# steineggerlab/Metabuli

Measured on AMD Instinct MI355X. Metric: Mreads/s classified (metabuli classify hot path, reads + index resident in HBM), higher is better.
Workload: dtype u64

## Files before the change

### include/mtb.h

```cpp
#ifndef MTB_H
#define MTB_H
#include <stddef.h>
#include <stdint.h>

#ifdef __cplusplus
extern "C" {
#endif

typedef enum {
    MTB_OK = 0,
    MTB_ERR_ARG = 1,
    MTB_ERR_IO = 2,
    MTB_ERR_DEVICE = 3,
    MTB_ERR_CAPACITY = 4,
    MTB_ERR_OOM = 5,
    MTB_ERR_UNSUPPORTED = 6
} mtb_status;

typedef struct { uint64_t value; uint64_t qinfo; } mtb_kmer;

typedef struct {
    uint64_t qinfo;
    int32_t  target_id;
    int32_t  species_id;
// ... 45 lines not shown
    uint32_t n_launch[MTB_NUM_KERNELS];
    uint64_t n_generic_reads;
    uint64_t n_slot_reads;
    uint64_t n_deferred_reads, n_many_reads, n_many_matches, n_many_kept;
    int32_t  join_variant, join_tuned;
    float    join_tune_ms[3];
    uint32_t join_tiles, join_tiles_windowed, join_tiles_outside;
} mtb_batch_stats;

typedef enum { MTB_JOIN_AUTO = 0, MTB_JOIN_Q1W6 = 1, MTB_JOIN_Q2W5 = 2, MTB_JOIN_WINDOW = 3 } mtb_join_variant;

const char *mtb_version(void);
const char *mtb_last_error(void);
void mtb_default_params(mtb_params *p);

mtb_status mtb_ctx_create(int device, void *stream, mtb_ctx **out);
void       mtb_ctx_destroy(mtb_ctx *);
mtb_status mtb_ctx_sync(mtb_ctx *);
mtb_status mtb_ctx_set_profiling(mtb_ctx *, int on);
mtb_status mtb_ctx_set_streams(mtb_ctx *, int n);
mtb_status mtb_ctx_set_workspace_limit(mtb_ctx *, uint64_t bytes);
mtb_status mtb_ctx_set_placement_probe(mtb_ctx *, int on);
mtb_status mtb_ctx_set_join_variant(mtb_ctx *, int variant);
mtb_status mtb_ctx_set_option(mtb_ctx *, const char *name, const char *value);
uint32_t   mtb_ctx_last_sub_batches(const mtb_ctx *);
uint64_t   mtb_ctx_last_scratch_bytes(const mtb_ctx *);

mtb_status mtb_index_open(mtb_ctx *, const char *dbdir, const char *taxonomy_dir,
                          mtb_params *params, mtb_index **out);
mtb_status mtb_index_open_stats(const mtb_index *, uint64_t *out4);
mtb_status mtb_index_from_device(mtb_ctx *, uint64_t *d_values, uint32_t *d_info,
                                 uint64_t n_targets, const char *taxonomy_dir,
                                 const int32_t *taxid_list, size_t n_taxids,
                                 const mtb_params *params, mtb_index **out);
mtb_status mtb_index_clone(mtb_index *src, mtb_ctx *dst_ctx, mtb_index **out);
typedef struct {
    uint8_t  values_handle[64], info_handle[64], dir_handle[64], dirbase_handle[64];
    uint64_t values_off, info_off, dir_off, dirbase_off;
    uint64_t n_targets;
    uint32_t dir_buckets, info_mask;
    int32_t  dir_depth, packed, has_info, match_last, device;
    int64_t  exporter_pid;
    uint64_t values_ptr, info_ptr, dir_ptr, dirbase_ptr;
} mtb_index_share;
mtb_status mtb_index_export(mtb_index *src, mtb_index_share *out);
mtb_status mtb_index_import(mtb_ctx *, const mtb_index_share *, const char *taxonomy_dir, const int32_t *taxid_list, size_t n_taxids,
// ... 164 lines not shown
```

### metabuli_amd/__init__.py

```python
from __future__ import annotations

import ctypes as C
import os
import subprocess

import numpy as np

_HERE = os.path.dirname(os.path.abspath(__file__))
_CSRC = os.path.join(_HERE, "csrc")
LIB_PATH = os.environ.get("MTB_LIB") or os.path.join(_CSRC, "libmtb.so")

kmer_dt = np.dtype([("value", "<u8"), ("qinfo", "<u8")])
match_dt = np.dtype([("qinfo", "<u8"), ("target_id", "<i4"), ("species_id", "<i4"), ("dna", "<u4"),
                     ("reh", "<u2"), ("ham", "u1"), ("pad", "u1")])
result_dt = np.dtype([("classification", "<i4"), ("score", "<f4"), ("qlen", "<i4"), ("qlen2", "<i4"),
                      ("is_classified", "u1"), ("flag", "u1"), ("n_taxcnt", "<u2"), ("taxcnt_off", "<u4")])

block_dt = np.dtype([("seq", "<u4"), ("strand", "<i4"), ("start", "<u8"), ("end", "<u8")])

MTB_OK, MTB_ERR_ARG, MTB_ERR_IO, MTB_ERR_DEVICE, MTB_ERR_CAPACITY, MTB_ERR_OOM, MTB_ERR_UNSUPPORTED = range(7)


class Params(C.Structure):
    _fields_ = [("seq_mode", C.c_int32), ("syncmer", C.c_int32), ("smer_len", C.c_int32),
# ... 112 lines not shown
        _chk(self.L.mtb_ctx_create(C.c_int(device), C.c_void_p(stream), C.byref(h)))
        self.h = h

    def close(self):
        if self.h:
            self.L.mtb_ctx_destroy(self.h)
            self.h = None

    def sync(self):
        _chk(self.L.mtb_ctx_sync(self.h))

    def set_profiling(self, on):
        _chk(self.L.mtb_ctx_set_profiling(self.h, C.c_int(1 if on else 0)))

    def set_placement_probe(self, on):
        _chk(self.L.mtb_ctx_set_placement_probe(self.h, C.c_int(1 if on else 0)))

    def set_workspace_limit(self, nbytes):
        _chk(self.L.mtb_ctx_set_workspace_limit(self.h, C.c_uint64(int(nbytes))))

    def set_join_variant(self, name):
        _chk(self.L.mtb_ctx_set_join_variant(self.h, C.c_int({"auto": 0, "q1w6": 1, "q2w5": 2, "window": 3}[name])))

    def set_option(self, name, value):
        _chk(self.L.mtb_ctx_set_option(self.h, name.encode(), None if value is None else str(value).encode()))

    @property
    def last_sub_batches(self):
        self.L.mtb_ctx_last_sub_batches.restype = C.c_uint32
        return int(self.L.mtb_ctx_last_sub_batches(self.h))

    @property
    def last_scratch_bytes(self):
        self.L.mtb_ctx_last_scratch_bytes.restype = C.c_uint64
        return int(self.L.mtb_ctx_last_scratch_bytes(self.h))

    def set_streams(self, n):
        _chk(self.L.mtb_ctx_set_streams(self.h, C.c_int(n)))

    def open_index(self, dbdir, params, taxonomy_dir=None):
        h = C.c_void_p()
        _chk(self.L.mtb_index_open(self.h, dbdir.encode(), taxonomy_dir.encode() if taxonomy_dir else None,
                                   C.byref(params), C.byref(h)))
        return Index(self, h)

    def clone_index(self, src):
# ... 461 lines not shown
```

### metabuli_amd/csrc/kernels_sort.h

```cpp
#ifndef MTB_KERNELS_SORT_H
#define MTB_KERNELS_SORT_H
#include "dev_util.h"
#include "kernels_scan.h"
#include "mtb_core.h"

#define MTB_SORT_TILE 2048
#ifndef MTB_SORT_ITEMS
#define MTB_SORT_ITEMS 8
#endif

template <int MODE>
__device__ __forceinline__ uint32_t radix_digit(uint64_t v, int shift) {
    if (MODE == 0) return (uint32_t)(v >> shift) & 255u;
    uint32_t two = (uint32_t)(v >> shift) & 1023u;
    uint32_t d = (two >> 5) * 21u + (two & 31u);
    return d < 511u ? d : 511u;
}

template <int NB, int MODE, int THREADS>
__global__ __launch_bounds__(THREADS) void k_radix_hist(const mtb_kmer *__restrict__ in, uint64_t n, int shift,
                                                         uint32_t *__restrict__ hist, uint32_t num_tiles) {
    __shared__ uint32_t s_h[NB];
    for (int b = threadIdx.x; b < NB; b += THREADS) s_h[b] = 0;
    __syncthreads();
    uint64_t base = (uint64_t)blockIdx.x * (THREADS * MTB_SORT_ITEMS);
#pragma unroll
    for (int r = 0; r < MTB_SORT_ITEMS; r++) {
        uint64_t i = base + (uint64_t)r * THREADS + threadIdx.x;
        if (i < n) atomicAdd(&s_h[radix_digit<MODE>(in[i].value, shift)], 1u);
    }
    __syncthreads();
    for (int b = threadIdx.x; b < NB; b += THREADS) hist[(uint64_t)b * num_tiles + blockIdx.x] = s_h[b];
}

#define MTB_HIST_GROUP 16
template <int NB, int THREADS, int TILE = THREADS * MTB_SORT_ITEMS>
__global__ __launch_bounds__(THREADS) void k_radix_hist_dig(const uint16_t *__restrict__ dig, uint64_t n, uint32_t *__restrict__ hist, uint32_t num_tiles) {
    static_assert(NB == THREADS, "one bin per thread");
    __shared__ uint32_t s_h[MTB_HIST_GROUP][NB];
    const uint32_t tile0 = blockIdx.x * MTB_HIST_GROUP;
#pragma unroll
    for (int g = 0; g < MTB_HIST_GROUP; g++) s_h[g][threadIdx.x] = 0;
    __syncthreads();
    for (int g = 0; g < MTB_HIST_GROUP; g++) {
        const uint64_t base = (uint64_t)(tile0 + g) * TILE;
        if (base >= n) break;
        if (TILE == THREADS * 8 && base + TILE <= n) {
            const uint4 q = *(const uint4 *)(dig + base + 8u * threadIdx.x);
            const uint32_t w[4] = {q.x, q.y, q.z, q.w};
#pragma unroll
            for (int k = 0; k < 4; k++) {
                const uint32_t d0 = w[k] & 0xFFFFu, d1 = w[k] >> 16;
                atomicAdd(&s_h[g][d0 < NB ? d0 : NB - 1], 1u);
                atomicAdd(&s_h[g][d1 < NB ? d1 : NB - 1], 1u);
            }
            continue;
        }
#pragma unroll
        for (int r = 0; r < TILE / THREADS; r++) {
            uint64_t i = base + (uint64_t)r * THREADS + threadIdx.x;
            if (i < n) { uint32_t d = dig[i]; atomicAdd(&s_h[g][d < NB ? d : NB - 1], 1u); }
        }
    }
    __syncthreads();
    uint32_t *row = hist + (uint64_t)threadIdx.x * num_tiles + tile0;
    if (tile0 + MTB_HIST_GROUP <= num_tiles && (((uint64_t)threadIdx.x * num_tiles + tile0) & 3u) == 0) {
#pragma unroll
        for (int g = 0; g < MTB_HIST_GROUP; g += 4) {
            uint4 v; v.x = s_h[g][threadIdx.x]; v.y = s_h[g + 1][threadIdx.x]; v.z = s_h[g + 2][threadIdx.x]; v.w = s_h[g + 3][threadIdx.x];
            *(uint4 *)(row + g) = v;
        }
    } else {
        for (int g = 0; g < MTB_HIST_GROUP && tile0 + g < num_tiles; g++) row[g] = s_h[g][threadIdx.x];
    }
}

#define MTB_SORT_NBKT 512
__device__ __forceinline__ uint32_t sort_tile_bucket(const uint32_t *__restrict__ first_tile, uint32_t t) {
    uint32_t lo = 0, hi = MTB_SORT_NBKT;
    while (hi - lo > 1) { const uint32_t mid = (lo + hi) >> 1; if (first_tile[mid] <= t) lo = mid; else hi = mid; }
    return lo;
}

template <int NB, int MODE, int THREADS>
__global__ __launch_bounds__(THREADS) void k_radix_scatter(const mtb_kmer *__restrict__ in, mtb_kmer *__restrict__ out,
                                                            uint64_t n, int shift, const uint32_t *__restrict__ tile_off,
                                                            uint32_t num_tiles, uint16_t *__restrict__ dig_out = nullptr, int next_shift = 0, int xcd_map = 1,
                                                            const uint32_t *__restrict__ plan = nullptr ) {
    constexpr int BITS = NB == 256 ? 8 : 9;
    constexpr int NW = THREADS / 64;
    constexpr int TILE = THREADS * MTB_SORT_ITEMS;
    static_assert(NB <= THREADS, "at least one thread per bin");
    __shared__ uint16_t s_cnt[NW][NB];
    __shared__ uint16_t s_start[NB];
    __shared__ uint32_t s_tmp[NW];
    __shared__ mtb_kmer s_buf[TILE];
    __shared__ uint32_t s_goff[NB];
    const uint32_t t = threadIdx.x, w = t >> 6, lane = t & 63u;
    if (plan) num_tiles = plan[513 + 512];
    const uint32_t per_xcd = (num_tiles + 7u) >> 3;
    const uint32_t tile = xcd_map ? (blockIdx.x & 7u) * per_xcd + (blockIdx.x >> 3) : blockIdx.x;
    if (tile >= num_tiles) return;
    uint64_t base = (uint64_t)tile * TILE;
    uint32_t my_off;
    if (plan) {
        const uint32_t *tfirst = plan + 513;
        const uint32_t b = sort_tile_bucket(tfirst, tile);
        const uint32_t j = tile - tfirst[b], ntb = tfirst[b + 1] - tfirst[b];
        base = (uint64_t)plan[b] + (uint64_t)j * TILE;
        n = plan[b + 1];
        my_off = t < NB ? tile_off[(uint64_t)512 * tfirst[b] + (uint64_t)t * ntb + j] : 0u;
    } else
    my_off = t < NB ? tile_off[(uint64_t)t * num_tiles + tile] : 0u;
    mtb_kmer e[MTB_SORT_ITEMS];
    uint32_t lrank[MTB_SORT_ITEMS];
    if (t < NB) {
#pragma unroll
        for (int k = 0; k < NW; k++) s_cnt[k][t] = 0;
    }
#pragma unroll
    for (int r = 0; r < MTB_SORT_ITEMS; r++) {
        uint64_t i = base + (uint64_t)w * (64 * MTB_SORT_ITEMS) + (uint64_t)r * 64 + lane;
        if (i < n) e[r] = in[i]; else { e[r].value = 0; e[r].qinfo = 0; }
    }
    __syncthreads();
#pragma unroll
    for (int r = 0; r < MTB_SORT_ITEMS; r++) {
        uint64_t i = base + (uint64_t)w * (64 * MTB_SORT_ITEMS) + (uint64_t)r * 64 + lane;
        bool valid = i < n;
        uint32_t d = radix_digit<MODE>(e[r].value, shift);
        uint64_t peers = __ballot(valid);
#pragma unroll
        for (int b = 0; b < BITS; b++) {
            bool bit = (d >> b) & 1u;
            uint64_t vote = __ballot(bit);
            peers &= bit ? vote : ~vote;
        }
        uint32_t rank_in_wave = (uint32_t)__popcll(peers & lanemask_lt());
        uint32_t before = s_cnt[w][d];
        __builtin_amdgcn_fence(__ATOMIC_ACQ_REL, "wavefront"); __builtin_amdgcn_wave_barrier();
        if (valid && rank_in_wave == 0) s_cnt[w][d] = (uint16_t)(before + (uint32_t)__popcll(peers));
        __builtin_amdgcn_fence(__ATOMIC_ACQ_REL, "wavefront"); __builtin_amdgcn_wave_barrier();
        lrank[r] = before + rank_in_wave;
    }
    __syncthreads();
    uint32_t run = 0;
    if (t < NB) {
#pragma unroll
        for (int k = 0; k < NW; k++) { uint32_t c = s_cnt[k][t]; s_cnt[k][t] = (uint16_t)run; run += c; }
    }
    uint32_t tot;
    uint32_t ex = block_exclusive_scan<uint32_t, NW>(run, s_tmp, &tot);
    if (t < NB) {
        s_start[t] = (uint16_t)ex;
        s_goff[t] = my_off - ex;
    }
    __syncthreads();
#pragma unroll
    for (int r = 0; r < MTB_SORT_ITEMS; r++) {
        uint64_t i = base + (uint64_t)w * (64 * MTB_SORT_ITEMS) + (uint64_t)r * 64 + lane;
        if (i < n) {
            uint32_t d = radix_digit<MODE>(e[r].value, shift);
            s_buf[(uint32_t)s_start[d] + s_cnt[w][d] + lrank[r]] = e[r];
        }
    }
    __syncthreads();
    uint32_t cnt = (uint32_t)((n - base) < TILE ? (n - base) : TILE);
    for (uint32_t i = t; i < cnt; i += THREADS) {
        mtb_kmer x = s_buf[i];
        uint32_t d = radix_digit<MODE>(x.value, shift);
        const uint64_t dst = (uint64_t)(s_goff[d] + i);
        out[dst] = x;
        if (dig_out) dig_out[dst] = (uint16_t)radix_digit<MODE>(x.value, next_shift);
    }
}

__global__ __launch_bounds__(512) void k_sort_plan(const uint32_t *__restrict__ scanned, uint32_t num_tiles, uint64_t n, uint32_t tile, uint32_t *__restrict__ plan) {
    __shared__ uint32_t s_tmp[8];
    const uint32_t b = threadIdx.x;
    const uint32_t start = scanned[(uint64_t)b * num_tiles];
    const uint32_t next = b + 1 < MTB_SORT_NBKT ? scanned[(uint64_t)(b + 1) * num_tiles] : (uint32_t)n;
    const uint32_t nt = (next - start + tile - 1) / tile;
    uint32_t tot;
    const uint32_t first = block_exclusive_scan<uint32_t, 8>(nt, s_tmp, &tot);
    plan[b] = start; plan[513 + b] = first;
    if (b == 0) { plan[512] = (uint32_t)n; plan[513 + 512] = tot; }
}
template <int NB, int THREADS, int TILE = THREADS * MTB_SORT_ITEMS>
__global__ __launch_bounds__(THREADS) void k_radix_hist_seg(const uint16_t *__restrict__ dig, const uint32_t *__restrict__ plan, uint32_t *__restrict__ hist) {
    static_assert(NB == THREADS, "one bin per thread");
    __shared__ uint32_t s_h[MTB_HIST_GROUP][NB];
    const uint32_t *bstart = plan, *tfirst = plan + 513;
    const uint32_t tiles = tfirst[512];
    const uint32_t tile0 = blockIdx.x * MTB_HIST_GROUP;
    if (tile0 >= tiles) return;
#pragma unroll
    for (int g = 0; g < MTB_HIST_GROUP; g++) s_h[g][threadIdx.x] = 0;
    __syncthreads();
    const uint32_t b0 = sort_tile_bucket(tfirst, tile0);
    uint32_t b = b0;
    for (int g = 0; g < MTB_HIST_GROUP; g++) {
        const uint32_t t = tile0 + g;
        if (t >= tiles) break;
        while (tfirst[b + 1] <= t) b++;
        const uint32_t base = bstart[b] + (t - tfirst[b]) * TILE;
        const uint32_t end = bstart[b + 1] < base + TILE ? bstart[b + 1] : base + TILE;
        if (TILE == THREADS * 8 && end == base + TILE && (base & 7u) == 0) {
            const uint4 q = *(const uint4 *)(dig + base + 8u * threadIdx.x);
            const uint32_t w[4] = {q.x, q.y, q.z, q.w};
#pragma unroll
            for (int k = 0; k < 4; k++) {
                const uint32_t d0 = w[k] & 0xFFFFu, d1 = w[k] >> 16;
                atomicAdd(&s_h[g][d0 < NB ? d0 : NB - 1], 1u);
                atomicAdd(&s_h[g][d1 < NB ? d1 : NB - 1], 1u);
            }
            continue;
        }
        const uint32_t a0 = base & ~7u;
        for (uint32_t ch = threadIdx.x; a0 + 8u * ch < end; ch += THREADS) {
            const uint32_t first = a0 + 8u * ch;
            const uint4 q = *(const uint4 *)(dig + first);
            const uint32_t w[4] = {q.x, q.y, q.z, q.w};
#pragma unroll
            for (int k = 0; k < 4; k++) {
                const uint32_t i0 = first + 2u * k, d0 = w[k] & 0xFFFFu, d1 = w[k] >> 16;
                if (i0 >= base && i0 < end) atomicAdd(&s_h[g][d0 < NB ? d0 : NB - 1], 1u);
                if (i0 + 1 >= base && i0 + 1 < end) atomicAdd(&s_h[g][d1 < NB ? d1 : NB - 1], 1u);
            }
        }
    }
    __syncthreads();
    const uint32_t last = tile0 + MTB_HIST_GROUP <= tiles ? tile0 + MTB_HIST_GROUP - 1 : tiles - 1;
    if (tfirst[b0 + 1] > last) {
        const uint32_t ntb = tfirst[b0 + 1] - tfirst[b0];
        uint32_t *row = hist + (uint64_t)512 * tfirst[b0] + (uint64_t)threadIdx.x * ntb + (tile0 - tfirst[b0]);
        for (uint32_t g = 0; g <= last - tile0; g++) row[g] = s_h[g][threadIdx.x];
    } else {
        uint32_t bb = b0;
        for (uint32_t g = 0; g <= last - tile0; g++) {
            const uint32_t t = tile0 + g;
            while (tfirst[bb + 1] <= t) bb++;
            const uint32_t ntb = tfirst[bb + 1] - tfirst[bb];
            hist[(uint64_t)512 * tfirst[bb] + (uint64_t)threadIdx.x * ntb + (t - tfirst[bb])] = s_h[g][threadIdx.x];
        }
    }
}

static inline uint64_t radix_hist_elems(uint64_t n, uint32_t bins = 256) { uint64_t tile = (uint64_t)bins * MTB_SORT_ITEMS; return (uint64_t)bins * ((n + tile - 1) / tile); }

static mtb_kmer *radix_sort_kmers(hipStream_t st, mtb_kmer *a, mtb_kmer *b, uint64_t n, int first_bit,
                                  uint32_t *hist, uint32_t *ws) {
    if (n == 0) return a;
    uint32_t tiles = (uint32_t)((n + MTB_SORT_TILE - 1) / MTB_SORT_TILE);
    mtb_kmer *src = a, *dst = b;
    for (int shift = first_bit; shift < 64; shift += 8) {
        hipLaunchKernelGGL((k_radix_hist<256, 0, 256>), dim3(tiles), dim3(256), 0, st, src, n, shift, hist, tiles);
        scan_launch<uint32_t, uint32_t, false>(st, hist, 256ull * tiles, false, hist, ws);
        hipLaunchKernelGGL((k_radix_scatter<256, 0, 256>), dim3((tiles + 7u) / 8u * 8u), dim3(256), 0, st, src, dst, n, shift, hist, tiles);
        mtb_kmer *tmp = src; src = dst; dst = tmp;
    }
    return src;
}

#endif
```

### metabuli_amd/csrc/mtb_api.hip

```cpp
#include <hip/hip_runtime.h>

#include <fcntl.h>
#include <limits.h>
#include <stdlib.h>
#include <sys/stat.h>
#include <unistd.h>

#include <atomic>
#include <chrono>
#include <condition_variable>
#include <mutex>
#include <functional>
#include <map>
#include <string>
#include <thread>
#include <vector>

#include "../../include/mtb.h"
#include "host_db.h"
#include "host/merge_plan.h"
#include "host/audit_plan.h"
#include "host/clade_filter.h"
#include "kernels_extract.h"
#include "kernels_extract_blocks.h"
// ... 90 lines not shown
    mtb_tables *d_tabs = nullptr;
    mtb_tables h_tabs;
    std::map<std::string, DevBuf> bufs;
    std::mutex bufs_mu;
    std::mutex reserve_mu;
    std::atomic<bool> reserve_cancel{false};
    uint64_t *d_scal = nullptr;
    unsigned long long *d_ovfctr = nullptr;
    uint64_t ovf_region = 0, ovf_max_region = 0;
    hipEvent_t ev[8];
    mtb_batch_stats stats;
    int profiling = 0;
    struct KEv { int id; hipEvent_t a, b; };
    std::vector<KEv> kev;
    std::vector<hipEvent_t> ev_pool;
    std::vector<mtb_ctx *> lanes;
    bool is_lane = false;
    uint32_t seg_epoch = 0;
    const void *seg_clean_p = nullptr; size_t seg_clean_cap = 0;
    double extract_yield = 0.0;
    uint64_t part_n_reads = 0; uint32_t part_max_len = 0;
    int part_mode = 0; uint32_t part_max_q = 0; uint64_t part_nk_real = 0;
    bool placement_probe = false;
    uint64_t ws_limit = 0;
    double ws_per_base = 0.0;
    uint64_t ws_max_sub_bases = 0;
    int ws_seq_mode = 0;
    uint32_t last_sub_batches = 0;
    bool fast_used = false;
    const mtb_kmer *last_sorted = nullptr; uint64_t last_sorted_n = 0;
    struct DeadSeg { char *p; size_t cap, used; };
    DeadSeg dead[3]; int n_dead = 0;
    uint64_t last_scratch_bytes = 0;
    hipStream_t copy_stream = nullptr; hipEvent_t copy_done[2] = {nullptr, nullptr};
    hipEvent_t unpacked[2] = {nullptr, nullptr};
    bool unpacked_rec[2] = {false, false};
    uint64_t prefetch_issued = 0, prefetch_used = 0;
    hipStream_t down_stream = nullptr; hipEvent_t down_ready = nullptr, down_done = nullptr; bool down_pending = false; int res_set = 0;
    int pk_set = 0;
    struct Prefetched { const void *key = nullptr, *key2 = nullptr; uint64_t n_reads = 0; bool valid = false; } pre[2];
    struct JoinTune { uint64_t key = 0; int calls = 0, pending = -1, best = -1; float ms[3] = {0.0f, 0.0f, 0.0f}; hipEvent_t e0 = nullptr, e1 = nullptr; } join_tunes[4]; uint32_t join_tune_next = 0;
    uint64_t many_stats[4] = {0, 0, 0, 0};
    uint32_t lslot_tf_start = 1;
    MtbOptions opt;
};
template <typename T> static T *scal(mtb_ctx *c, Scal s) { return (T *)(c->d_scal + s); }
// ... 255 lines not shown
mtb_status mtb_ctx_set_placement_probe(mtb_ctx *c, int on) {
    if (!c) return fail(MTB_ERR_ARG, "NULL ctx");
    c->placement_probe = on != 0;
    for (mtb_ctx *l : c->lanes) l->placement_probe = on != 0;
    return MTB_OK;
}
mtb_status mtb_ctx_set_workspace_limit(mtb_ctx *c, uint64_t bytes) {
    if (!c) return fail(MTB_ERR_ARG, "NULL ctx");
    c->ws_limit = bytes;
    for (mtb_ctx *l : c->lanes) l->ws_limit = bytes;
    return MTB_OK;
}
mtb_status mtb_ctx_set_option(mtb_ctx *c, const char *name, const char *value) {
    if (!c || !name) return fail(MTB_ERR_ARG, "NULL ctx / name");
    if (!mtbopt::set(&c->opt, name, value)) return fail(MTB_ERR_ARG, std::string("unknown switch or bad value: ") + name + "=" + (value ? value : "(unset)"));
    for (mtb_ctx *l : c->lanes) l->opt = c->opt;
    return MTB_OK;
}
mtb_status mtb_ctx_set_join_variant(mtb_ctx *c, int variant) {
    static const char *const names[] = {"auto", "q1w6", "q2w5", "window"};
    if (!c || variant < 0 || variant > 3) return fail(MTB_ERR_ARG, "variant must be MTB_JOIN_AUTO .. MTB_JOIN_WINDOW");
    return mtb_ctx_set_option(c, "MTB_JOIN_VARIANT", names[variant]);
}
uint32_t mtb_ctx_last_sub_batches(const mtb_ctx *c) { return c ? c->last_sub_batches : 0; }
uint64_t mtb_ctx_last_scratch_bytes(const mtb_ctx *c) { return c ? c->last_scratch_bytes : 0; }
mtb_status mtb_ctx_set_streams(mtb_ctx *c, int n) {
    if (!c || n < 1 || n > 8) return fail(MTB_ERR_ARG, "streams must be 1..8");
    HIPCHK(hipSetDevice(c->device));
    while ((int)c->lanes.size() > (n == 1 ? 0 : n)) { mtb_ctx_destroy(c->lanes.back()); c->lanes.pop_back(); }
    while (n > 1 && (int)c->lanes.size() < n) {
        mtb_ctx *l = new mtb_ctx();
        l->device = c->device; l->is_lane = true; l->d_tabs = c->d_tabs; l->h_tabs = c->h_tabs; l->profiling = c->profiling; l->placement_probe = c->placement_probe; l->opt = c->opt;
        HIPCHK(hipStreamCreateWithFlags(&l->stream, hipStreamNonBlocking));
        HIPCHK(hipMalloc((void **)&l->d_scal, SC_WORDS * sizeof(uint64_t)));
        HIPCHK(hipMalloc((void **)&l->d_ovfctr, MTB_OVF_STRIPES * 64));
        for (int i = 0; i < 8; i++) HIPCHK(hipEventCreate(&l->ev[i]));
        memset(&l->stats, 0, sizeof(l->stats));
        c->lanes.push_back(l);
    }
    return MTB_OK;
}

}

static mtb_status d2h(mtb_ctx *c, void *dst, const void *src, size_t bytes) {
    HIPCHK(hipMemcpyAsync(dst, src, bytes, hipMemcpyDeviceToHost, c->stream));
    HIPCHK(hipStreamSynchronize(c->stream));
    return MTB_OK;
}
static mtb_status h2d(mtb_ctx *c, void *dst, const void *src, size_t bytes) {
    if (bytes == 0) return MTB_OK;
    HIPCHK(hipMemcpyAsync(dst, src, bytes, hipMemcpyHostToDevice, c->stream));
    HIPCHK(hipStreamSynchronize(c->stream));
    return MTB_OK;
}
// ... 74 lines not shown
    uint32_t *d_cnt; uint64_t *d_koff; uint64_t *d_ws;
    STCHK(ensure(c, "counts", n_reads, &d_cnt)); STCHK(ensure(c, "koff", n_reads + 1, &d_koff));
    STCHK(ensure(c, "scanws", scan_ws_elems(n_reads + 1), &d_ws));
    { KTimer kt(c, MTB_K_EXTRACT_COUNT);
    hipLaunchKernelGGL((k_extract<0>), dim3(grid), dim3(64), 0, c->stream, a, c->d_tabs, d_cnt, (const uint64_t *)nullptr,
                       (mtb_kmer *)nullptr, d_qlen, d_qlen2, scal<uint32_t>(c, SC_MAX_LEN), (unsigned long long *)nullptr, (uint64_t)0); }
    { KTimer kt(c, MTB_K_SCAN); scan_launch<uint32_t, uint64_t, false>(c->stream, d_cnt, n_reads, true, d_koff, d_ws); }
    uint64_t total = 0;
    STCHK(d2h(c, &total, d_koff + n_reads, 8));
    if (opt.want_max_len) { uint64_t ml = 0; STCHK(d2h(c, &ml, scal<uint64_t>(c, SC_MAX_LEN), 8)); ex->max_len = (uint32_t)ml; }
    if (total >= (1ull << 32)) return fail(MTB_ERR_ARG, "more than 2^32-1 query metamers in one batch; split the batch");
    mtb_kmer *d_k;
    STCHK(ensure(c, "kmersA", total, &d_k));
    if (total) { KTimer kt(c, MTB_K_EXTRACT_EMIT);
        hipLaunchKernelGGL((k_extract<1>), dim3(grid), dim3(64), 0, c->stream, a, c->d_tabs, (uint32_t *)nullptr,
                           (const uint64_t *)d_koff, d_k, (int32_t *)nullptr, (int32_t *)nullptr, (uint32_t *)nullptr,
                           (unsigned long long *)nullptr, (uint64_t)0); }
    HIPCHK(hipGetLastError());
    ex->d_k = d_k; ex->nk = ex->nk_real = total;
    return MTB_OK;
}

#define MTB_SORT_AA6 (-6)
static mtb_status dev_sort(mtb_ctx *c, mtb_kmer *d_a, uint64_t n, int first_bit, mtb_kmer **sorted, uint16_t *d_dig, int aa_first_shift) {
    *sorted = d_a;
    if (n == 0) return MTB_OK;
    const bool aa = first_bit == MTB_SORT_AA6;
    const uint32_t bins = aa ? 512u : 256u;
    mtb_kmer *d_b; uint32_t *d_hist; uint64_t *d_ws;
    STCHK(ensure(c, "kmersB", n, &d_b));
    STCHK(ensure(c, "hist", radix_hist_elems(n, bins), &d_hist));
    STCHK(ensure(c, "scanws", scan_ws_elems(radix_hist_elems(n, bins)), &d_ws));
    {
        const int xcd_map = c->opt.sort_no_xcd ? 0 : 1;
        const uint32_t sc_threads = aa ? 512u : 256u;
        const uint64_t tile = (uint64_t)sc_threads * MTB_SORT_ITEMS;
        uint32_t tiles = (uint32_t)((n + tile - 1) / tile);
        mtb_kmer *src = d_a, *dst = d_b;
        uint16_t *dig_src = aa ? d_dig : nullptr, *dig_dst = nullptr;
        if (dig_src) STCHK(ensure(c, "digB", n + 8, &dig_dst));
        if (aa && dig_src && aa_first_shift == 34 && sort_msd_first(c)) {
            uint32_t *d_plan;
            STCHK(ensure(c, "sortplan", 1026, &d_plan));
            const uint32_t seg_tiles_max = tiles + MTB_SORT_NBKT;
            STCHK(ensure(c, "hist", (uint64_t)bins * seg_tiles_max, &d_hist));
            STCHK(ensure(c, "scanws", scan_ws_elems((uint64_t)bins * seg_tiles_max), &d_ws));
            { KTimer kt(c, MTB_K_RADIX_HIST);
              hipLaunchKernelGGL((k_radix_hist_dig<512, 512>), dim3((tiles + MTB_HIST_GROUP - 1) / MTB_HIST_GROUP), dim3(512), 0, c->stream, (const uint16_t *)dig_src, n, d_hist, tiles); }
            { KTimer kt(c, MTB_K_SCAN); scan_launch<uint32_t, uint32_t, false>(c->stream, d_hist, (uint64_t)bins * tiles, false, d_hist, (uint32_t *)d_ws); }
            hipLaunchKernelGGL(k_sort_plan, dim3(1), dim3(512), 0, c->stream, (const uint32_t *)d_hist, tiles, n, (uint32_t)tile, d_plan);
            { KTimer kt(c, MTB_K_RADIX_SCATTER);
              hipLaunchKernelGGL((k_radix_scatter<512, 1, 512>), dim3((tiles + 7u) / 8u * 8u), dim3(512), 0, c->stream, (const mtb_kmer *)src, dst, n, 54, (const uint32_t *)d_hist, tiles, dig_dst, 34, xcd_map); }
            { mtb_kmer *tmp = src; src = dst; dst = tmp; uint16_t *t2 = dig_src; dig_src = dig_dst; dig_dst = t2; }
            for (int shift = 34; shift <= 44; shift += 10) {
                const dim3 hg((seg_tiles_max + MTB_HIST_GROUP - 1) / MTB_HIST_GROUP), sg((seg_tiles_max + 7u) / 8u * 8u);
                { KTimer kt(c, MTB_K_RADIX_HIST);
                  hipLaunchKernelGGL((k_radix_hist_seg<512, 512>), hg, dim3(512), 0, c->stream, (const uint16_t *)dig_src, (const uint32_t *)d_plan, d_hist); }
                { KTimer kt(c, MTB_K_SCAN); scan_launch<uint32_t, uint32_t, false>(c->stream, d_hist, (uint64_t)bins * seg_tiles_max, false, d_hist, (uint32_t *)d_ws); }
                { KTimer kt(c, MTB_K_RADIX_SCATTER);
                  hipLaunchKernelGGL((k_radix_scatter<512, 1, 512>), sg, dim3(512), 0, c->stream, (const mtb_kmer *)src, dst, n, shift, (const uint32_t *)d_hist, tiles,
                                     shift == 34 ? dig_dst : (uint16_t *)nullptr, 44, xcd_map, (const uint32_t *)d_plan); }
                { mtb_kmer *tmp = src; src = dst; dst = tmp; uint16_t *t2 = dig_src; dig_src = dig_dst; dig_dst = t2; }
            }
            *sorted = src;
            HIPCHK(hipGetLastError());
            return MTB_OK;
        }
        for (int shift = aa ? aa_first_shift : first_bit; shift < 64; shift += aa ? 10 : 8) {
            { KTimer kt(c, MTB_K_RADIX_HIST);
              const dim3 hg((tiles + MTB_HIST_GROUP - 1) / MTB_HIST_GROUP);
              if (aa && dig_src) hipLaunchKernelGGL((k_radix_hist_dig<512, 512>), hg, dim3(512), 0, c->stream, (const uint16_t *)dig_src, n, d_hist, tiles);
              else if (aa) hipLaunchKernelGGL((k_radix_hist<512, 1, 512>), dim3(tiles), dim3(512), 0, c->stream, (const mtb_kmer *)src, n, shift, d_hist, tiles);
              else hipLaunchKernelGGL((k_radix_hist<256, 0, 256>), dim3(tiles), dim3(256), 0, c->stream, (const mtb_kmer *)src, n, shift, d_hist, tiles); }
            { KTimer kt(c, MTB_K_SCAN); scan_launch<uint32_t, uint32_t, false>(c->stream, d_hist, (uint64_t)bins * tiles, false, d_hist, (uint32_t *)d_ws); }
            { KTimer kt(c, MTB_K_RADIX_SCATTER);
              const dim3 sg((tiles + 7u) / 8u * 8u);
              uint16_t *dnext = (dig_src && shift + 10 < 64) ? dig_dst : (uint16_t *)nullptr;
              if (aa) hipLaunchKernelGGL((k_radix_scatter<512, 1, 512>), sg, dim3(512), 0, c->stream, (const mtb_kmer *)src, dst, n, shift, (const uint32_t *)d_hist, tiles, dnext, shift + 10, xcd_map);
              else hipLaunchKernelGGL((k_radix_scatter<256, 0, 256>), sg, dim3(256), 0, c->stream, (const mtb_kmer *)src, dst, n, shift, (const uint32_t *)d_hist, tiles); }
            mtb_kmer *tmp = src; src = dst; dst = tmp;
            if (dig_src) { uint16_t *t2 = dig_src; dig_src = dig_dst; dig_dst = t2; }
        }
        *sorted = src;
    }
    HIPCHK(hipGetLastError());
    return MTB_OK;
}

struct IndexUse;
static mtb_dir_view dir_view(const mtb_index *ix);
static mtb_index_view index_view(const mtb_index *ix) {
    mtb_index_view v;
    v.values = ix->d_values; v.info = ix->d_info; v.n_targets = ix->T; v.tax2species = ix->d_tax2species;
    v.max_taxid = ix->tax.max_id; v.info_mask = ix->info_mask; v.kmer_format = ix->params.kmer_format;
    return v;
}
static mtb_tax_view tax_view(const mtb_index *ix) {
    mtb_tax_view v;
    v.acc_leaf = ix->d_accleaf; v.canon = ix->d_canon; v.parent = ix->d_parent; v.depth = ix->d_depth; v.under_euk = ix->d_under; v.sp_parent = ix->d_spparent;
    v.max_taxid = ix->tax.max_id;
    v.node = ix->d_node;
// ... 2185 lines not shown
    {
        mtb_status sd = build_directory(c, sl);
        if (sd != MTB_OK) { mtb_index_close(sl); return sd; }
    }
    *out = sl;
    return MTB_OK;
}

mtb_status mtb_part_extract(mtb_ctx *c, const mtb_params *p, const char *d_bases, const uint64_t *d_offs, const char *d_bases2,
                            const uint64_t *d_offs2, uint64_t n_reads, const uint64_t *bounds, uint32_t n_parts, const mtb_kmer **d_sorted,
                            uint64_t *n_kmers, uint64_t *part_counts, uint64_t *part_starts) {
    if (!c || !p || !d_offs || !bounds || !d_sorted || !n_kmers || !part_counts || n_parts == 0) return fail(MTB_ERR_ARG, "NULL argument");
    HIPCHK(hipSetDevice(c->device));
    *d_sorted = nullptr; *n_kmers = 0;
    for (uint32_t q = 0; q < n_parts; q++) { part_counts[q] = 0; if (part_starts) part_starts[q] = 0; }
    c->part_n_reads = n_reads; c->part_max_len = 0; c->part_mode = 0; c->part_max_q = 0; c->part_nk_real = 0;
    if (n_reads == 0) return MTB_OK;
    int32_t *d_ql, *d_ql2;
    STCHK(ensure(c, "qlen", n_reads, &d_ql)); STCHK(ensure(c, "qlen2", n_reads, &d_ql2));
    mtb_kmer *d_s; Extracted ex; const Reads rd{d_bases, d_offs, d_bases2, d_offs2, n_reads};
    if (part_starts && p->seq_mode != 3 && !c->opt.part_exact) {
        const bool aa6 = p->kmer_format == 2;
        ExtractOpts tagged; tagged.single_pass = true; tagged.tag_ordinals = true; tagged.want_digits = aa6;
        STCHK(dev_extract(c, p, rd, d_ql, d_ql2, tagged, &ex));
        const uint64_t nk = ex.nk;
        if (ex.max_len + 3 < MTB_SLOT_MAX_POS && ex.max_q <= 384) {
            const int low_bits = aa6 ? 34 : 32;
            STCHK(dev_sort(c, ex.d_k, ex.nk, aa6 ? MTB_SORT_AA6 : 32, &d_s, ex.d_dig,  34));
            c->part_max_len = ex.max_len; c->part_mode = 1; c->part_max_q = ex.max_q; c->part_nk_real = ex.nk_real;
            std::vector<uint64_t> key(2 * n_parts), pos(2 * n_parts);
            for (uint32_t q = 0; q < n_parts; q++) {
                const uint64_t pre = bounds[q] >> low_bits;
                key[2 * q] = pre << low_bits;
                key[2 * q + 1] = pre + 1 >= (1ull << (64 - low_bits)) ? UINT64_MAX : (pre + 1) << low_bits;
            }
            if (nk) STCHK(lower_bounds(c, (const uint64_t *)d_s, nk, 2, key.data(), 2 * n_parts, pos.data()));
            for (uint32_t q = 0; q < n_parts; q++) {
                const uint64_t lo = q == 0 ? 0 : pos[2 * q];
                const uint64_t hi = q + 1 < n_parts ? (key[2 * (q + 1) + 1] == UINT64_MAX ? nk : pos[2 * (q + 1) + 1]) : nk;
                part_starts[q] = lo; part_counts[q] = hi > lo ? hi - lo : 0;
            }
            *d_sorted = d_s; *n_kmers = nk;
            return MTB_OK;
        }
    }
    STCHK(dev_extract(c, p, rd, d_ql, d_ql2,  ExtractOpts(), &ex));
    const uint64_t nk = ex.nk;
    STCHK(dev_sort(c, ex.d_k, ex.nk, 24, &d_s,  nullptr, 0));
    c->part_max_len = ex.max_len;
    std::vector<uint64_t> pos(n_parts);
    if (nk) STCHK(lower_bounds(c, (const uint64_t *)d_s, nk, 2, bounds, n_parts, pos.data()));
// ... 1194 lines not shown
```

Baseline: 70.64.

## Process multiple stages per radix scatter tile to double tile size

Adds a ROUNDS template parameter to the radix scatter and histogram kernels so that each block ranks twice as many keys (16-bit packed local ranks) and then writes them out in staged passes through the same shared buffer. This is on by default (rounds=2) for the AA6 digit-assisted sort path. The aim is to halve the number of tiles, which shrinks the histogram and scan work and lengthens the contiguous output runs per bin. In exchange it raises per-thread register use and adds extra barriers between stages. It also adds a sort_rounds API knob and profiling timers around the partitioned extract and sort.

```diff
diff --git a/include/mtb.h b/include/mtb.h
--- a/include/mtb.h
+++ b/include/mtb.h
@@ -91,6 +91,7 @@
 mtb_status mtb_ctx_set_workspace_limit(mtb_ctx *, uint64_t bytes);
 mtb_status mtb_ctx_set_placement_probe(mtb_ctx *, int on);
 mtb_status mtb_ctx_set_join_variant(mtb_ctx *, int variant);
+mtb_status mtb_ctx_set_sort_rounds(mtb_ctx *, int rounds);
 mtb_status mtb_ctx_set_option(mtb_ctx *, const char *name, const char *value);
 uint32_t   mtb_ctx_last_sub_batches(const mtb_ctx *);
 uint64_t   mtb_ctx_last_scratch_bytes(const mtb_ctx *);
diff --git a/metabuli_amd/__init__.py b/metabuli_amd/__init__.py
--- a/metabuli_amd/__init__.py
+++ b/metabuli_amd/__init__.py
@@ -158,6 +158,9 @@
     def set_join_variant(self, name):
         _chk(self.L.mtb_ctx_set_join_variant(self.h, C.c_int({"auto": 0, "q1w6": 1, "q2w5": 2, "window": 3}[name])))
 
+    def set_sort_rounds(self, rounds):
+        _chk(self.L.mtb_ctx_set_sort_rounds(self.h, C.c_int(int(rounds))))
+
     def set_option(self, name, value):
         _chk(self.L.mtb_ctx_set_option(self.h, name.encode(), None if value is None else str(value).encode()))
 
diff --git a/metabuli_amd/csrc/kernels_sort.h b/metabuli_amd/csrc/kernels_sort.h
--- a/metabuli_amd/csrc/kernels_sort.h
+++ b/metabuli_amd/csrc/kernels_sort.h
@@ -45,14 +45,19 @@
     for (int g = 0; g < MTB_HIST_GROUP; g++) {
         const uint64_t base = (uint64_t)(tile0 + g) * TILE;
         if (base >= n) break;
-        if (TILE == THREADS * 8 && base + TILE <= n) {
-            const uint4 q = *(const uint4 *)(dig + base + 8u * threadIdx.x);
-            const uint32_t w[4] = {q.x, q.y, q.z, q.w};
-#pragma unroll
-            for (int k = 0; k < 4; k++) {
-                const uint32_t d0 = w[k] & 0xFFFFu, d1 = w[k] >> 16;
-                atomicAdd(&s_h[g][d0 < NB ? d0 : NB - 1], 1u);
-                atomicAdd(&s_h[g][d1 < NB ? d1 : NB - 1], 1u);
+        if (TILE % (THREADS * 8) == 0 && base + TILE <= n) {
+            uint4 q[TILE / (THREADS * 8)];
+#pragma unroll
+            for (int j = 0; j < TILE / (THREADS * 8); j++) q[j] = *(const uint4 *)(dig + base + (uint64_t)j * (THREADS * 8) + 8u * threadIdx.x);
+#pragma unroll
+            for (int j = 0; j < TILE / (THREADS * 8); j++) {
+                const uint32_t w[4] = {q[j].x, q[j].y, q[j].z, q[j].w};
+#pragma unroll
+                for (int k = 0; k < 4; k++) {
+                    const uint32_t d0 = w[k] & 0xFFFFu, d1 = w[k] >> 16;
+                    atomicAdd(&s_h[g][d0 < NB ? d0 : NB - 1], 1u);
+                    atomicAdd(&s_h[g][d1 < NB ? d1 : NB - 1], 1u);
+                }
             }
             continue;
         }
@@ -82,20 +87,24 @@
     return lo;
 }
 
-template <int NB, int MODE, int THREADS>
-__global__ __launch_bounds__(THREADS) void k_radix_scatter(const mtb_kmer *__restrict__ in, mtb_kmer *__restrict__ out,
+template <int NB, int MODE, int THREADS, int ROUNDS = 1>
+__global__ __launch_bounds__(THREADS, ROUNDS == 2 ? 2 * THREADS / 256 : 1 ) void k_radix_scatter(const mtb_kmer *__restrict__ in, mtb_kmer *__restrict__ out,
                                                             uint64_t n, int shift, const uint32_t *__restrict__ tile_off,
                                                             uint32_t num_tiles, uint16_t *__restrict__ dig_out = nullptr, int next_shift = 0, int xcd_map = 1,
                                                             const uint32_t *__restrict__ plan = nullptr ) {
     constexpr int BITS = NB == 256 ? 8 : 9;
     constexpr int NW = THREADS / 64;
-    constexpr int TILE = THREADS * MTB_SORT_ITEMS;
+    constexpr int IT = MTB_SORT_ITEMS * ROUNDS;
+    constexpr int STAGE = THREADS * MTB_SORT_ITEMS;
+    constexpr int TILE = STAGE * ROUNDS;
     static_assert(NB <= THREADS, "at least one thread per bin");
+    static_assert(ROUNDS >= 1 && TILE <= 12288, "s_cnt and s_start hold tile-local positions in 16 bits");
     __shared__ uint16_t s_cnt[NW][NB];
     __shared__ uint16_t s_start[NB];
     __shared__ uint32_t s_tmp[NW];
-    __shared__ mtb_kmer s_buf[TILE];
+    __shared__ mtb_kmer s_buf[STAGE];
     __shared__ uint32_t s_goff[NB];
+    __shared__ int s_shift;
     const uint32_t t = threadIdx.x, w = t >> 6, lane = t & 63u;
     if (plan) num_tiles = plan[513 + 512];
     const uint32_t per_xcd = (num_tiles + 7u) >> 3;
@@ -112,22 +121,23 @@
         my_off = t < NB ? tile_off[(uint64_t)512 * tfirst[b] + (uint64_t)t * ntb + j] : 0u;
     } else
     my_off = t < NB ? tile_off[(uint64_t)t * num_tiles + tile] : 0u;
-    mtb_kmer e[MTB_SORT_ITEMS];
-    uint32_t lrank[MTB_SORT_ITEMS];
+    const uint64_t i0 = base + (uint64_t)w * (64 * IT) + lane;
+    const mtb_kmer *__restrict__ first = in + i0;
+    const uint32_t mine = i0 < n ? (uint32_t)(n - i0 < TILE ? n - i0 : TILE) : 0u;
+    mtb_kmer e[IT];
+    uint32_t lrank[ROUNDS == 1 ? IT : IT / 2];
     if (t < NB) {
 #pragma unroll
         for (int k = 0; k < NW; k++) s_cnt[k][t] = 0;
     }
 #pragma unroll
-    for (int r = 0; r < MTB_SORT_ITEMS; r++) {
-        uint64_t i = base + (uint64_t)w * (64 * MTB_SORT_ITEMS) + (uint64_t)r * 64 + lane;
-        if (i < n) e[r] = in[i]; else { e[r].value = 0; e[r].qinfo = 0; }
-    }
-    __syncthreads();
-#pragma unroll
-    for (int r = 0; r < MTB_SORT_ITEMS; r++) {
-        uint64_t i = base + (uint64_t)w * (64 * MTB_SORT_ITEMS) + (uint64_t)r * 64 + lane;
-        bool valid = i < n;
+    for (int r = 0; r < IT; r++) {
+        if ((uint32_t)r * 64u < mine) e[r] = first[r * 64]; else { e[r].value = 0; e[r].qinfo = 0; }
+    }
+    __syncthreads();
+#pragma unroll
+    for (int r = 0; r < IT; r++) {
+        bool valid = (uint32_t)r * 64u < mine;
         uint32_t d = radix_digit<MODE>(e[r].value, shift);
         uint64_t peers = __ballot(valid);
 #pragma unroll
@@ -141,7 +151,9 @@
         __builtin_amdgcn_fence(__ATOMIC_ACQ_REL, "wavefront"); __builtin_amdgcn_wave_barrier();
         if (valid && rank_in_wave == 0) s_cnt[w][d] = (uint16_t)(before + (uint32_t)__popcll(peers));
         __builtin_amdgcn_fence(__ATOMIC_ACQ_REL, "wavefront"); __builtin_amdgcn_wave_barrier();
-        lrank[r] = before + rank_in_wave;
+        if (ROUNDS == 1) lrank[r] = before + rank_in_wave;
+        else if (r & 1) lrank[r >> 1] |= (before + rank_in_wave) << 16;
+        else lrank[r >> 1] = before + rank_in_wave;
     }
     __syncthreads();
     uint32_t run = 0;
@@ -154,24 +166,52 @@
     if (t < NB) {
         s_start[t] = (uint16_t)ex;
         s_goff[t] = my_off - ex;
-    }
-    __syncthreads();
-#pragma unroll
-    for (int r = 0; r < MTB_SORT_ITEMS; r++) {
-        uint64_t i = base + (uint64_t)w * (64 * MTB_SORT_ITEMS) + (uint64_t)r * 64 + lane;
-        if (i < n) {
-            uint32_t d = radix_digit<MODE>(e[r].value, shift);
-            s_buf[(uint32_t)s_start[d] + s_cnt[w][d] + lrank[r]] = e[r];
-        }
-    }
-    __syncthreads();
-    uint32_t cnt = (uint32_t)((n - base) < TILE ? (n - base) : TILE);
-    for (uint32_t i = t; i < cnt; i += THREADS) {
-        mtb_kmer x = s_buf[i];
-        uint32_t d = radix_digit<MODE>(x.value, shift);
-        const uint64_t dst = (uint64_t)(s_goff[d] + i);
-        out[dst] = x;
-        if (dig_out) dig_out[dst] = (uint16_t)radix_digit<MODE>(x.value, next_shift);
+        if (ROUNDS > 1) {
+#pragma unroll
+            for (int k = 0; k < NW; k++) s_cnt[k][t] += (uint16_t)ex;
+        }
+    }
+    if (ROUNDS > 1 && t == 0) s_shift = shift;
+    __syncthreads();
+    const uint32_t cnt = (uint32_t)((n - base) < TILE ? (n - base) : TILE);
+    if (ROUNDS > 1) {
+        const int shift_again = s_shift;
+#pragma unroll
+        for (int r = 0; r < IT; r++) {
+            uint32_t d = radix_digit<MODE>(e[r].value, shift_again);
+            const uint32_t rk = (r & 1) ? lrank[r >> 1] >> 16 : lrank[r >> 1] & 0xFFFFu;
+            const uint32_t p = (uint32_t)r * 64u < mine ? s_cnt[w][d] + rk : 0xFFFFu;
+            lrank[r >> 1] = (r & 1) ? (lrank[r >> 1] & 0xFFFFu) | (p << 16) : (lrank[r >> 1] & 0xFFFF0000u) | p;
+        }
+    }
+#pragma unroll
+    for (int q = 0; q < ROUNDS; q++) {
+        const uint32_t lo = (uint32_t)q * STAGE;
+        if (q > 0) {
+            if (lo >= cnt) break;
+            __syncthreads();
+        }
+#pragma unroll
+        for (int r = 0; r < IT; r++) {
+            if (ROUNDS == 1) {
+                if ((uint32_t)r * 64u < mine) {
+                    uint32_t d = radix_digit<MODE>(e[r].value, shift);
+                    s_buf[(uint32_t)s_start[d] + s_cnt[w][d] + lrank[r]] = e[r];
+                }
+            } else {
+                const uint32_t p = ((r & 1) ? lrank[r >> 1] >> 16 : lrank[r >> 1] & 0xFFFFu) - lo;
+                if (p < (uint32_t)STAGE) s_buf[p] = e[r];
+            }
+        }
+        __syncthreads();
+        const uint32_t hi = cnt - lo < (uint32_t)STAGE ? cnt - lo : (uint32_t)STAGE;
+        for (uint32_t i = t; i < hi; i += THREADS) {
+            mtb_kmer x = s_buf[i];
+            uint32_t d = radix_digit<MODE>(x.value, shift);
+            const uint64_t dst = (uint64_t)(s_goff[d] + lo + i);
+            out[dst] = x;
+            if (dig_out) dig_out[dst] = (uint16_t)radix_digit<MODE>(x.value, next_shift);
+        }
     }
 }
 
@@ -205,14 +245,19 @@
         while (tfirst[b + 1] <= t) b++;
         const uint32_t base = bstart[b] + (t - tfirst[b]) * TILE;
         const uint32_t end = bstart[b + 1] < base + TILE ? bstart[b + 1] : base + TILE;
-        if (TILE == THREADS * 8 && end == base + TILE && (base & 7u) == 0) {
-            const uint4 q = *(const uint4 *)(dig + base + 8u * threadIdx.x);
-            const uint32_t w[4] = {q.x, q.y, q.z, q.w};
-#pragma unroll
-            for (int k = 0; k < 4; k++) {
-                const uint32_t d0 = w[k] & 0xFFFFu, d1 = w[k] >> 16;
-                atomicAdd(&s_h[g][d0 < NB ? d0 : NB - 1], 1u);
-                atomicAdd(&s_h[g][d1 < NB ? d1 : NB - 1], 1u);
+        if (TILE % (THREADS * 8) == 0 && end == base + TILE && (base & 7u) == 0) {
+            uint4 q[TILE / (THREADS * 8)];
+#pragma unroll
+            for (int j = 0; j < TILE / (THREADS * 8); j++) q[j] = *(const uint4 *)(dig + base + (uint32_t)j * (THREADS * 8) + 8u * threadIdx.x);
+#pragma unroll
+            for (int j = 0; j < TILE / (THREADS * 8); j++) {
+                const uint32_t w[4] = {q[j].x, q[j].y, q[j].z, q[j].w};
+#pragma unroll
+                for (int k = 0; k < 4; k++) {
+                    const uint32_t d0 = w[k] & 0xFFFFu, d1 = w[k] >> 16;
+                    atomicAdd(&s_h[g][d0 < NB ? d0 : NB - 1], 1u);
+                    atomicAdd(&s_h[g][d1 < NB ? d1 : NB - 1], 1u);
+                }
             }
             continue;
         }
@@ -246,7 +291,7 @@
     }
 }
 
-static inline uint64_t radix_hist_elems(uint64_t n, uint32_t bins = 256) { uint64_t tile = (uint64_t)bins * MTB_SORT_ITEMS; return (uint64_t)bins * ((n + tile - 1) / tile); }
+static inline uint64_t radix_hist_elems(uint64_t n, uint32_t bins = 256, uint32_t rounds = 1) { uint64_t tile = (uint64_t)bins * MTB_SORT_ITEMS * rounds; return (uint64_t)bins * ((n + tile - 1) / tile); }
 
 static mtb_kmer *radix_sort_kmers(hipStream_t st, mtb_kmer *a, mtb_kmer *b, uint64_t n, int first_bit,
                                   uint32_t *hist, uint32_t *ws) {
diff --git a/metabuli_amd/csrc/mtb_api.hip b/metabuli_amd/csrc/mtb_api.hip
--- a/metabuli_amd/csrc/mtb_api.hip
+++ b/metabuli_amd/csrc/mtb_api.hip
@@ -136,6 +136,7 @@
     uint64_t part_n_reads = 0; uint32_t part_max_len = 0;
     int part_mode = 0; uint32_t part_max_q = 0; uint64_t part_nk_real = 0;
     bool placement_probe = false;
+    int sort_rounds = 0;
     uint64_t ws_limit = 0;
     double ws_per_base = 0.0;
     uint64_t ws_max_sub_bases = 0;
@@ -437,6 +438,12 @@
     if (!c || variant < 0 || variant > 3) return fail(MTB_ERR_ARG, "variant must be MTB_JOIN_AUTO .. MTB_JOIN_WINDOW");
     return mtb_ctx_set_option(c, "MTB_JOIN_VARIANT", names[variant]);
 }
+mtb_status mtb_ctx_set_sort_rounds(mtb_ctx *c, int rounds) {
+    if (!c || rounds < 0 || rounds > 3) return fail(MTB_ERR_ARG, "sort rounds must be 0 (default) or 1 .. 3");
+    c->sort_rounds = rounds;
+    for (mtb_ctx *l : c->lanes) l->sort_rounds = rounds;
+    return MTB_OK;
+}
 uint32_t mtb_ctx_last_sub_batches(const mtb_ctx *c) { return c ? c->last_sub_batches : 0; }
 uint64_t mtb_ctx_last_scratch_bytes(const mtb_ctx *c) { return c ? c->last_scratch_bytes : 0; }
 mtb_status mtb_ctx_set_streams(mtb_ctx *c, int n) {
@@ -445,7 +452,7 @@
     while ((int)c->lanes.size() > (n == 1 ? 0 : n)) { mtb_ctx_destroy(c->lanes.back()); c->lanes.pop_back(); }
     while (n > 1 && (int)c->lanes.size() < n) {
         mtb_ctx *l = new mtb_ctx();
-        l->device = c->device; l->is_lane = true; l->d_tabs = c->d_tabs; l->h_tabs = c->h_tabs; l->profiling = c->profiling; l->placement_probe = c->placement_probe; l->opt = c->opt;
+        l->device = c->device; l->is_lane = true; l->d_tabs = c->d_tabs; l->h_tabs = c->h_tabs; l->profiling = c->profiling; l->placement_probe = c->placement_probe; l->sort_rounds = c->sort_rounds; l->opt = c->opt;
         HIPCHK(hipStreamCreateWithFlags(&l->stream, hipStreamNonBlocking));
         HIPCHK(hipMalloc((void **)&l->d_scal, SC_WORDS * sizeof(uint64_t)));
         HIPCHK(hipMalloc((void **)&l->d_ovfctr, MTB_OVF_STRIPES * 64));
@@ -566,19 +573,25 @@
 }
 
 #define MTB_SORT_AA6 (-6)
+#define MTB_SORT_ROUNDS_DEFAULT 2
+#define MTB_BY_SORT_ROUNDS(rounds, ...) do { switch (rounds) { \
+    case 3: { constexpr int R = 3; __VA_ARGS__; } break; \
+    case 2: { constexpr int R = 2; __VA_ARGS__; } break; \
+    default: { constexpr int R = 1; __VA_ARGS__; } break; } } while (0)
 static mtb_status dev_sort(mtb_ctx *c, mtb_kmer *d_a, uint64_t n, int first_bit, mtb_kmer **sorted, uint16_t *d_dig, int aa_first_shift) {
     *sorted = d_a;
     if (n == 0) return MTB_OK;
     const bool aa = first_bit == MTB_SORT_AA6;
     const uint32_t bins = aa ? 512u : 256u;
+    const int rounds = aa && d_dig ? (c->sort_rounds ? c->sort_rounds : MTB_SORT_ROUNDS_DEFAULT) : 1;
     mtb_kmer *d_b; uint32_t *d_hist; uint64_t *d_ws;
     STCHK(ensure(c, "kmersB", n, &d_b));
-    STCHK(ensure(c, "hist", radix_hist_elems(n, bins), &d_hist));
-    STCHK(ensure(c, "scanws", scan_ws_elems(radix_hist_elems(n, bins)), &d_ws));
+    STCHK(ensure(c, "hist", radix_hist_elems(n, bins, rounds), &d_hist));
+    STCHK(ensure(c, "scanws", scan_ws_elems(radix_hist_elems(n, bins, rounds)), &d_ws));
     {
         const int xcd_map = c->opt.sort_no_xcd ? 0 : 1;
         const uint32_t sc_threads = aa ? 512u : 256u;
-        const uint64_t tile = (uint64_t)sc_threads * MTB_SORT_ITEMS;
+        const uint64_t tile = (uint64_t)sc_threads * MTB_SORT_ITEMS * rounds;
         uint32_t tiles = (uint32_t)((n + tile - 1) / tile);
         mtb_kmer *src = d_a, *dst = d_b;
         uint16_t *dig_src = aa ? d_dig : nullptr, *dig_dst = nullptr;
@@ -590,20 +603,20 @@
             STCHK(ensure(c, "hist", (uint64_t)bins * seg_tiles_max, &d_hist));
             STCHK(ensure(c, "scanws", scan_ws_elems((uint64_t)bins * seg_tiles_max), &d_ws));
             { KTimer kt(c, MTB_K_RADIX_HIST);
-              hipLaunchKernelGGL((k_radix_hist_dig<512, 512>), dim3((tiles + MTB_HIST_GROUP - 1) / MTB_HIST_GROUP), dim3(512), 0, c->stream, (const uint16_t *)dig_src, n, d_hist, tiles); }
+              MTB_BY_SORT_ROUNDS(rounds, hipLaunchKernelGGL((k_radix_hist_dig<512, 512, 512 * MTB_SORT_ITEMS * R>), dim3((tiles + MTB_HIST_GROUP - 1) / MTB_HIST_GROUP), dim3(512), 0, c->stream, (const uint16_t *)dig_src, n, d_hist, tiles)); }
             { KTimer kt(c, MTB_K_SCAN); scan_launch<uint32_t, uint32_t, false>(c->stream, d_hist, (uint64_t)bins * tiles, false, d_hist, (uint32_t *)d_ws); }
             hipLaunchKernelGGL(k_sort_plan, dim3(1), dim3(512), 0, c->stream, (const uint32_t *)d_hist, tiles, n, (uint32_t)tile, d_plan);
             { KTimer kt(c, MTB_K_RADIX_SCATTER);
-              hipLaunchKernelGGL((k_radix_scatter<512, 1, 512>), dim3((tiles + 7u) / 8u * 8u), dim3(512), 0, c->stream, (const mtb_kmer *)src, dst, n, 54, (const uint32_t *)d_hist, tiles, dig_dst, 34, xcd_map); }
+              MTB_BY_SORT_ROUNDS(rounds, hipLaunchKernelGGL((k_radix_scatter<512, 1, 512, R>), dim3((tiles + 7u) / 8u * 8u), dim3(512), 0, c->stream, (const mtb_kmer *)src, dst, n, 54, (const uint32_t *)d_hist, tiles, dig_dst, 34, xcd_map, (const uint32_t *)nullptr)); }
             { mtb_kmer *tmp = src; src = dst; dst = tmp; uint16_t *t2 = dig_src; dig_src = dig_dst; dig_dst = t2; }
             for (int shift = 34; shift <= 44; shift += 10) {
                 const dim3 hg((seg_tiles_max + MTB_HIST_GROUP - 1) / MTB_HIST_GROUP), sg((seg_tiles_max + 7u) / 8u * 8u);
                 { KTimer kt(c, MTB_K_RADIX_HIST);
-                  hipLaunchKernelGGL((k_radix_hist_seg<512, 512>), hg, dim3(512), 0, c->stream, (const uint16_t *)dig_src, (const uint32_t *)d_plan, d_hist); }
+                  MTB_BY_SORT_ROUNDS(rounds, hipLaunchKernelGGL((k_radix_hist_seg<512, 512, 512 * MTB_SORT_ITEMS * R>), hg, dim3(512), 0, c->stream, (const uint16_t *)dig_src, (const uint32_t *)d_plan, d_hist)); }
                 { KTimer kt(c, MTB_K_SCAN); scan_launch<uint32_t, uint32_t, false>(c->stream, d_hist, (uint64_t)bins * seg_tiles_max, false, d_hist, (uint32_t *)d_ws); }
                 { KTimer kt(c, MTB_K_RADIX_SCATTER);
-                  hipLaunchKernelGGL((k_radix_scatter<512, 1, 512>), sg, dim3(512), 0, c->stream, (const mtb_kmer *)src, dst, n, shift, (const uint32_t *)d_hist, tiles,
-                                     shift == 34 ? dig_dst : (uint16_t *)nullptr, 44, xcd_map, (const uint32_t *)d_plan); }
+                  MTB_BY_SORT_ROUNDS(rounds, hipLaunchKernelGGL((k_radix_scatter<512, 1, 512, R>), sg, dim3(512), 0, c->stream, (const mtb_kmer *)src, dst, n, shift, (const uint32_t *)d_hist, tiles,
+                                     shift == 34 ? dig_dst : (uint16_t *)nullptr, 44, xcd_map, (const uint32_t *)d_plan)); }
                 { mtb_kmer *tmp = src; src = dst; dst = tmp; uint16_t *t2 = dig_src; dig_src = dig_dst; dig_dst = t2; }
             }
             *sorted = src;
@@ -613,14 +626,15 @@
         for (int shift = aa ? aa_first_shift : first_bit; shift < 64; shift += aa ? 10 : 8) {
             { KTimer kt(c, MTB_K_RADIX_HIST);
               const dim3 hg((tiles + MTB_HIST_GROUP - 1) / MTB_HIST_GROUP);
-              if (aa && dig_src) hipLaunchKernelGGL((k_radix_hist_dig<512, 512>), hg, dim3(512), 0, c->stream, (const uint16_t *)dig_src, n, d_hist, tiles);
+              if (aa && dig_src) MTB_BY_SORT_ROUNDS(rounds, hipLaunchKernelGGL((k_radix_hist_dig<512, 512, 512 * MTB_SORT_ITEMS * R>), hg, dim3(512), 0, c->stream, (const uint16_t *)dig_src, n, d_hist, tiles));
               else if (aa) hipLaunchKernelGGL((k_radix_hist<512, 1, 512>), dim3(tiles), dim3(512), 0, c->stream, (const mtb_kmer *)src, n, shift, d_hist, tiles);
               else hipLaunchKernelGGL((k_radix_hist<256, 0, 256>), dim3(tiles), dim3(256), 0, c->stream, (const mtb_kmer *)src, n, shift, d_hist, tiles); }
             { KTimer kt(c, MTB_K_SCAN); scan_launch<uint32_t, uint32_t, false>(c->stream, d_hist, (uint64_t)bins * tiles, false, d_hist, (uint32_t *)d_ws); }
             { KTimer kt(c, MTB_K_RADIX_SCATTER);
               const dim3 sg((tiles + 7u) / 8u * 8u);
               uint16_t *dnext = (dig_src && shift + 10 < 64) ? dig_dst : (uint16_t *)nullptr;
-              if (aa) hipLaunchKernelGGL((k_radix_scatter<512, 1, 512>), sg, dim3(512), 0, c->stream, (const mtb_kmer *)src, dst, n, shift, (const uint32_t *)d_hist, tiles, dnext, shift + 10, xcd_map);
+              if (aa && dig_src) MTB_BY_SORT_ROUNDS(rounds, hipLaunchKernelGGL((k_radix_scatter<512, 1, 512, R>), sg, dim3(512), 0, c->stream, (const mtb_kmer *)src, dst, n, shift, (const uint32_t *)d_hist, tiles, dnext, shift + 10, xcd_map, (const uint32_t *)nullptr));
+              else if (aa) hipLaunchKernelGGL((k_radix_scatter<512, 1, 512>), sg, dim3(512), 0, c->stream, (const mtb_kmer *)src, dst, n, shift, (const uint32_t *)d_hist, tiles, (uint16_t *)nullptr, shift + 10, xcd_map);
               else hipLaunchKernelGGL((k_radix_scatter<256, 0, 256>), sg, dim3(256), 0, c->stream, (const mtb_kmer *)src, dst, n, shift, (const uint32_t *)d_hist, tiles); }
             mtb_kmer *tmp = src; src = dst; dst = tmp;
             if (dig_src) { uint16_t *t2 = dig_src; dig_src = dig_dst; dig_dst = t2; }
@@ -2852,11 +2866,19 @@
     if (part_starts && p->seq_mode != 3 && !c->opt.part_exact) {
         const bool aa6 = p->kmer_format == 2;
         ExtractOpts tagged; tagged.single_pass = true; tagged.tag_ordinals = true; tagged.want_digits = aa6;
+        if (c->profiling) { collect_kernel_times(c); memset(&c->stats, 0, sizeof(c->stats)); HIPCHK(hipEventRecord(c->ev[0], c->stream)); }
         STCHK(dev_extract(c, p, rd, d_ql, d_ql2, tagged, &ex));
         const uint64_t nk = ex.nk;
         if (ex.max_len + 3 < MTB_SLOT_MAX_POS && ex.max_q <= 384) {
             const int low_bits = aa6 ? 34 : 32;
+            if (c->profiling) HIPCHK(hipEventRecord(c->ev[1], c->stream));
             STCHK(dev_sort(c, ex.d_k, ex.nk, aa6 ? MTB_SORT_AA6 : 32, &d_s, ex.d_dig,  34));
+            if (c->profiling) {
+                HIPCHK(hipEventRecord(c->ev[2], c->stream)); HIPCHK(hipEventSynchronize(c->ev[2]));
+                HIPCHK(hipEventElapsedTime(&c->stats.ms_extract, c->ev[0], c->ev[1])); HIPCHK(hipEventElapsedTime(&c->stats.ms_sort, c->ev[1], c->ev[2]));
+                collect_kernel_times(c);
+                c->stats.n_reads = n_reads; c->stats.n_bases = ex.n_bases; c->stats.n_kmers = ex.nk_real;
+            }
             c->part_max_len = ex.max_len; c->part_mode = 1; c->part_max_q = ex.max_q; c->part_nk_real = ex.nk_real;
             std::vector<uint64_t> key(2 * n_parts), pos(2 * n_parts);
             for (uint32_t q = 0; q < n_parts; q++) {
```

After: 69.92. 0.99x the previous value.
